# Genomics-HSE/VGsim

Measured on AMD Instinct MI355X. Metric: simulated events/sec (direct + tau-leap) at 1/2/4/8 MI355X vs Cython CPU, higher is better.
Workload: dtype f64; 1 GPU; BASELINE config 3: 65536 haplotypes (8 sites) x 64 populations x 1 susceptibility group, direct Gillespie, bit-exact mode (PCG64 stream, reference summation order), index-case start, b=2.5 d=0.9 s=0.1 m=0.01/site, total migration 0.01, N=1e7; replicates_per_gpu=16384, events_per_replicate=100000, trajectory_points=1001

## Files before the change

vgsim_amd/csrc/vgx_quad.hip:

```cpp
#include <hip/hip_runtime.h>
#include <stdint.h>
#include <vector>
#include "vgx_dev.h"
#include "vgx_rng.h"
#include "vgx_wave.h"
#include "vgx_rowprim.h"
#include "vgx_rowlist.h"
#include "vgx_flat.h"

#ifndef VGX_QUAD_WAVES
#define VGX_QUAD_WAVES 2
#endif

#ifdef VGX_PROFILE
#define QPROF(i)                                                        \
    do {                                                                \
        unsigned long long prof_t1 = __builtin_readcyclecounter();      \
        prof_acc[i] += prof_t1 - prof_t0;                               \
        prof_t0 = prof_t1;                                              \
    } while (0)
#else
#define QPROF(i)
#endif

// ... 226 lines not shown
}

extern "C" __global__ void __launch_bounds__(64) vgx_quad_prep_kernel(VgxDevParams p, const double *cd, double *effMig,
                                                                     double *maxEBM, int32_t *has_mig) {
    const int P = p.P;
    bool anyf = false;
    for (int base = 0; base < P; base += 64) {
        const int pn2 = base + (int)threadIdx.x;
        double mx = 0.0;
        if (pn2 < P) {
            const double *m2 = p.mig + (int64_t)pn2 * P;
            for (int pn1 = 0; pn1 < P; ++pn1) {
                if (pn1 == pn2) continue;
                const double *m1 = p.mig + (int64_t)pn1 * P;
                double e = 0.0;
                for (int pn3 = 0; pn3 < P; ++pn3) e += m1[pn3] * m2[pn3] * cd[pn3] / p.actualSizes[pn3];
                effMig[(int64_t)pn1 * P + pn2] = e;
                if (e > mx) mx = e;
            }
            maxEBM[pn2] = mx * p.maxEffectiveBirth;
        }
        anyf = anyf || (__ballot(pn2 < P && mx * p.maxEffectiveBirth != 0.0) != 0ull);
    }
    if (threadIdx.x == 0) *has_mig = anyf ? 1 : 0;
}
extern "C" __attribute__((visibility("hidden"))) hipError_t vgxi_launch_quad_prep(const VgxDevParams *p, const double *cd, double *effMig,
                                                                                 double *maxEBM, int32_t *has_mig, hipStream_t stream) {
    hipLaunchKernelGGL(vgx_quad_prep_kernel, dim3(1), dim3(64), 0, stream, *p, cd, effMig, maxEBM, has_mig);
    return hipGetLastError();
}

struct VgxQuadKArgs { VgxDirectArgs a; QArgs qa; };
typedef const VgxQuadKArgs __attribute__((address_space(4))) *QuadKA;
template <int QT, bool RCPDIV>
static __device__ __forceinline__ void quad_body() {
    const QuadKA ka = (QuadKA)__builtin_amdgcn_kernarg_segment_ptr();
    const auto &a = ka->a;
    const auto &qa = ka->qa;
    const int lane = threadIdx.x, row = lane >> 4, rl = lane & 15;
    const auto &p = a.p;
    const auto &r = a.r;
    const int P = p.P, sites = p.sites, H = p.H;
    const int64_t R = a.n_replicates;
    const int64_t rep_raw = (int64_t)blockIdx.x * 4 + row;
    const bool live = rep_raw < R;
    const int64_t rep = live ? rep_raw : R - 1;
    const int nslot = (P + 15) >> 4;
    const bool has_mig = qa.has_mig[0] != 0;

    extern __shared__ __attribute__((aligned(16))) unsigned char smem[];
    double *k_cd = (double *)smem, *k_as = k_cd + 64, *k_smul = k_as + 64, *k_mebm = k_smul + 64, *k_rcp = k_mebm + 64;
    uint64_t *k_jump = (uint64_t *)(smem + Q_CONST_BYTES) + rl * 4;
    unsigned char *blk = smem + Q_CONST_BYTES + Q_RNG_BYTES + row * Q_REP_BYTES;
    double *s_inf = (double *)blk, *s_bc = s_inf + 64;
    double *s_ts = s_bc + 64, *s_ti = s_ts + 64;
    int32_t *s_nocc = (int32_t *)(s_ti + 64);
    double *s_cc = (double *)(s_nocc + 64);
    int64_t *s_cnt = (int64_t *)(s_cc + 4);
    uint64_t *s_inc = (uint64_t *)(s_cnt + 6);
    int32_t *s_zero = (int32_t *)(s_inc + 2);
    uint32_t *s_stage = (uint32_t *)(s_zero + 64);
    int stage_n = 0;
    int64_t stage_slot0 = 0;
    auto stage_flush = [&](bool f) {
        WSYNC();
        if (f && live) {
            const int n6 = stage_n * 6;
            int32_t *c = r.ev_cols + (rep * r.evcap + stage_slot0) * VGX_EV_COLS;
            uint32_t *q = (uint32_t *)(r.ev_rate + rep * r.evcap + stage_slot0);
#pragma unroll
            for (int j = 0; j < 3; ++j)
                if (rl + 16 * j < n6) c[rl + 16 * j] = (int32_t)s_stage[rl + 16 * j];
            if (rl < 2 * stage_n) q[rl] = s_stage[48 + rl];
        }
        if (f) stage_n = 0;
        WSYNC();
    };
#define QBUMP(i) do { if (rl == 0) s_cnt[i] += 1; } while (0)

    const double c_b = p.cb_b[0], c_sig = p.cb_sigma[0], c_d = p.c_d[0], c_s = p.c_s[0], c_tm = p.c_tm[0];

    {
        const double *gD = r.popD + rep * PD_COUNT * P;
        const int64_t *gI64 = r.popI + rep * PI_COUNT * P;
        const int32_t *gN = r.nocc + rep * P;
        const int pn = lane;
        k_cd[pn] = pn < P ? gD[PD_CD * P + pn] : 0.0;
        k_as[pn] = pn < P ? p.actualSizes[pn] : 1.0;
        k_rcp[pn] = pn < P ? 1.0 / p.actualSizes[pn] : 1.0;
        k_smul[pn] = pn < P ? c_s * p.sampMult[pn] : 0.0;
        k_mebm[pn] = pn < P ? qa.maxEBM[pn] : 0.0;
        for (int s = 0; s < 4; ++s) {
            const int pq = s * 16 + rl;
            const bool ok = pq < P;
            s_inf[pq] = 0.0; s_bc[pq] = 0.0;
            if (rl < 4) s_cc[rl] = 0.0;
            s_ts[pq] = ok ? (double)gI64[PI_TOTSUS * P + pq] : 0.0;
            s_ti[pq] = ok ? (double)gI64[PI_TOTINF * P + pq] : 0.0;
            s_nocc[pq] = ok ? gN[pq] : 0;
            s_zero[pq] = QT < 4 && ok ? gN[pq] : 0;
        }
    }
    WSYNC();

    const int64_t cap = r.cap, capT = r.capT;
    int32_t *lhap = r.lhap + rep * P * cap;
    int32_t *lcls = r.lcls + rep * P * cap;
    int64_t *lcnt = r.lcnt + rep * P * cap;
    int32_t *lcnt32 = r.lcnt32 + rep * P * cap;
#define L8(pop) ((uint8_t *)(r.lcnt32 + R * P * cap) + (rep * P + (int64_t)(pop)) * cap)
#define B8(v) ((uint8_t)((v) < 255 ? (v) : 255))
    int64_t *ltsum = r.ltsum + rep * P * capT;
    const bool has_traj = r.traj != nullptr;
    const VgxRepScalars *sc = r.sc + rep;
    if (QT < 4) {
        for (int pn = 0; pn < P; ++pn) q_zero_tail(lcnt32 + (int64_t)pn * cap, s_nocc[pn], cap, live);
        WSYNC();
    }

    double t_now = sc->currentTime, totalRate = 0.0, totalMig = 0.0;
    double gI = (double)sc->globalInfectious;
    int64_t ev_ptr = sc->ev_ptr;
    int64_t cS = sc->sCounter;
    if (rl == 0) {
        s_cnt[QC_B] = sc->bCounter; s_cnt[QC_D] = sc->dCounter; s_cnt[QC_M] = sc->mCounter;
        s_cnt[QC_MIGP] = sc->migPlus; s_cnt[QC_MIGN] = sc->migNonPlus;
    }
    int64_t loops = 0, att_loops = 0, good_attempt = sc->good_attempt;
    int att = 0, restarts = 0, last_att = -1, traj_next = 0;
    int st = live ? ST_REBUILD : ST_DONE, err = 0;
    bool open = false;
    const double tlimit = (double)a.time;
    const bool has_tl = !(a.time == -1.0f);

    if (row == 0) {
        const uint64_t MH = 0x2360ED051FC65DA4ull, ML = 0x4385DF649FCCF645ull;
        uint64_t Ah = MH, Al = ML, Gh = 0, Gl = 1;
        for (int j = 1; j < 16; ++j) {
            uint64_t nh, nl, gh, gl;
            vgx_mul128(Ah, Al, MH, ML, nh, nl);
            vgx_mul128(Gh, Gl, MH, ML, gh, gl);
            vgx_add128(gh, gl, 0, 1);
            if (j <= rl) { Ah = nh; Al = nl; Gh = gh; Gl = gl; }
        }
        k_jump[0] = Ah; k_jump[1] = Al; k_jump[2] = Gh; k_jump[3] = Gl;
    }
    WSYNC();
    uint64_t g_sh = 0, g_sl = 0;
    double g_val = 0.0;
    int pos = 8;
    int32_t ch_cn[4] = {0, 0, 0, 0};
    double tc = 0.0;
    int tc_pi = -1;

#ifdef VGX_PROFILE
    unsigned long long prof_acc[VGX_PROF_SLOTS], prof_t0 = __builtin_readcyclecounter();
    for (int i = 0; i < VGX_PROF_SLOTS; ++i) prof_acc[i] = 0;
    int prof_tiles[13] = {0, 0, 0, 0, 0, 0, 0, 0, 0, 0, 0, 0, 0};
#endif
    while (true) {
        QPROF(0);
        const bool run = st != ST_DONE;
        if (!__ballot(run)) break;
        const bool rebuild = st == ST_REBUILD;

        bool end_attempt = false, ev = false;
        if (st == ST_RUN) {
            if (!open) {
                if (att >= a.attempts) {
                    st = ST_DONE;
                } else {
                    VgxPcg64 sd;
                    vgx_pcg64_seed(sd, (uint64_t)r.seeds[rep], (uint32_t)att);
                    g_sh = sd.sh; g_sl = sd.sl;
                    if (rl == 0) { s_inc[0] = sd.ih; s_inc[1] = sd.il; }
                    pos = 8;
                    open = true;
                    last_att = att; att_loops = 0;
                    if (!(totalRate + totalMig != 0.0 && gI != 0.0)) end_attempt = true;
                }
            }
            if (st == ST_RUN && !end_attempt &&
                !(ev_ptr < a.ev_size && (a.sample_size == -1 || cS <= a.sample_size) && (!has_tl || t_now < tlimit)))
                end_attempt = true;
            if (st == ST_RUN && !end_attempt) {
                if (loops >= a.max_loop) { err = Q_ERR_LOOP_GUARD; st = ST_DONE; }
                else ev = true;
            }
        }

        int u_lo = 0, u_hi = rebuild ? P : 0;
        int op_n = 0, op_pi = 0, op_h0 = 0, op_h1 = 0;
        int op_d0 = 0;
        int e_type = -1, e_hap = 0, e_pop = 0, e_nh = 0, e_np = 0;
        double den = 0.0;
        int ch_pi = -1;
        double m_pre[4] = {0.0, 0.0, 0.0, 0.0};
        int pm_pi = -1;

        QPROF(1);
        if (__ballot(ev)) {
            if (__builtin_expect(__ballot(ev && pos == 8) != 0, 0)) {
                const bool fill = ev && pos == 8;
                uint64_t h, l, ch, cl;
                vgx_mul128(k_jump[0], k_jump[1], g_sh, g_sl, h, l);
                vgx_mul128(k_jump[2], k_jump[3], s_inc[0], s_inc[1], ch, cl);
                vgx_add128(h, l, ch, cl);
                const double u = vgx_pcg64_output_double(h, l);
                const double v = (rl & 1) ? u : -vgx_log(u);
                const uint64_t nh = (uint64_t)rowget_i64((int64_t)h, 15), nl = (uint64_t)rowget_i64((int64_t)l, 15);
                if (fill) { g_val = v; g_sh = nh; g_sl = nl; pos = 0; }
            }
            const int pp = min(pos, 7);
            const double nlog = rowget_f64(g_val, 2 * pp), u2 = rowget_f64(g_val, 2 * pp + 1);
            if (ev) { pos += 1; loops += 1; att_loops += 1; }
            QPROF(2);
            den = totalRate + totalMig;
            const double t_new = t_now + (nlog / den);
            if (has_traj) {
                while (true) {
                    const double tg = r.traj_t0 + (double)traj_next * r.traj_dt;
                    const bool emit = ev && live && traj_next < r.traj_points && tg < t_new;
                    if (__builtin_expect(!__ballot(emit), 1)) break;
                    if (emit) {
                        double *o = r.traj + (rep * r.traj_points + traj_next) * (int64_t)P * 2;
                        for (int s = 0; s < nslot; ++s) {
                            const int pn = s * 16 + rl;
                            if (pn < P) { o[pn * 2 + 0] = s_ti[pn]; o[pn * 2 + 1] = s_ts[pn]; }
                        }
                        traj_next += 1;
                    }
                }
            }
            if (ev) t_now = t_new;

            QPROF(3);
            double rn = u2;
            const double choose0 = rn * den;
            double choose = choose0;
            const bool evn = ev && (totalRate > choose);
            const bool evm = ev && !evn;

            int pi = 0;
            {
                rn = choose / totalRate;
                const double rr_ = totalRate * rn;
                const double c0 = s_cc[0], c1 = s_cc[1], c2 = s_cc[2], c3 = s_cc[3];
                const int slot = !(c0 < rr_) ? 0 : !(c1 < rr_) ? 1 : !(c2 < rr_) ? 2 : 3;
                const bool any = !(c3 < rr_);
                const double cin = slot == 0 ? 0.0 : slot == 1 ? c0 : slot == 2 ? c1 : c2;
                const double w = s_inf[slot * 16 + rl];
                double tot_;
                const double pre = row_scan16(w, cin, tot_);
                const int q = row_min(any && slot * 16 + rl < P && !(pre < rr_) ? rl : 16);
                double total, wi;
                if (q < 16) { pi = slot * 16 + q; total = rowget_f64(pre, q); wi = rowget_f64(w, q); }
                else { pi = P - 1; total = c3; wi = s_inf[P - 1]; }
                if (evn && wi == 0.0) err = Q_ERR_ZERO_WEIGHT + 256 * 1;
                rn = (rr_ - (total - wi)) / wi;
                choose = rn * wi;
            }
            const double infect_pi = s_inf[pi];
            rn = (choose - 0.0) / infect_pi;
            const double bC = s_bc[pi];
            const double smul = k_smul[pi];
            const double tE = ((bC + c_d) + smul) + c_tm;
            const int n_sel = evn ? s_nocc[pi] : 0;
            const int32_t *lh = lhap + (int64_t)pi * cap;
            int32_t *l3 = lcnt32 + (int64_t)pi * cap;
            int64_t *lt = ltsum + (int64_t)pi * capT;
            {
                const double *mrow = p.mig + (int64_t)pi * P;
#pragma unroll
                for (int s = 0; s < 4; ++s)
                    if (s < nslot) m_pre[s] = mrow[min(s * 16 + rl, P - 1)];
                pm_pi = evn ? pi : -1;
            }

            QPROF(4);
            const double r2 = infect_pi * rn;
            int k_hit = -1;
            double pre_hit = 0.0, w_hit = 0.0;
            int hap_hit = 0;
            int64_t cnt_hit = 0;
            const int maxn = rows_max(n_sel);
            if (__builtin_expect(maxn <= 64, QT < 4)) {
                const int nch = (maxn + 15) >> 4;
                const int last = max(n_sel - 1, 0);
                const double tEz = n_sel > 0 ? tE : 0.0;
                int32_t cn4[4];
                int hp4[4];
                double w4[4];
#pragma unroll
                for (int c = 0; c < 4; ++c) {
                    cn4[c] = 0; hp4[c] = 0; w4[c] = 0.0;
                    if (c < nch) {
                        const int k = c * 16 + rl;
                        hp4[c] = lh[min(k, last)];
                        if (QT < 4 && c > 0) {
                            cn4[c] = l3[k];
                            w4[c] = tEz * (double)cn4[c];
                        } else {
                            cn4[c] = l3[min(k, last)];
                            w4[c] = k < n_sel ? tE * (double)cn4[c] : 0.0;
                        }
                    }
                }
                double carry = 0.0, carry_hit = 0.0;
                int c_hit = nch == 1 ? 0 : -1;
                if (nch > 1) {
#pragma unroll
                    for (int c = 0; c < 4; ++c) {
                        if (c < nch) {
                            const double acc = row_sum16(w4[c], carry);
                            if (c_hit < 0 && c * 16 < n_sel && !(acc < r2)) { c_hit = c; carry_hit = carry; }
                            carry = acc;
                        }
                    }
                }
                const int cc = c_hit >= 0 ? c_hit : (last >> 4);
                const double w = cc == 0 ? w4[0] : cc == 1 ? w4[1] : cc == 2 ? w4[2] : w4[3];
                const int32_t cn = cc == 0 ? cn4[0] : cc == 1 ? cn4[1] : cc == 2 ? cn4[2] : cn4[3];
                const int hp = cc == 0 ? hp4[0] : cc == 1 ? hp4[1] : cc == 2 ? hp4[2] : hp4[3];
                double tot_;
                const double pre = row_scan16(w, c_hit >= 0 ? carry_hit : 0.0, tot_);
                if (nch == 1) carry = tot_;
                const int q = row_min(c_hit >= 0 && cc * 16 + rl < n_sel && !(pre < r2) ? rl : 16);
                const int qq = q < 16 ? q : (last & 15);
                pre_hit = q < 16 ? rowget_f64(pre, qq) : carry;
                w_hit = rowget_f64(w, qq);
                hap_hit = rowget_i32(hp, qq); cnt_hit = rowget_i32(cn, qq);
                if (q < 16) k_hit = cc * 16 + q;
                else if (evn) {
                    if (n_sel > 0 && hap_hit == H - 1 && (QT < 4 || cnt_hit != 0)) k_hit = n_sel - 1; else err = Q_ERR_ZERO_WEIGHT + 256 * 2;
                }
                if (evn) {
#pragma unroll
                    for (int c = 0; c < 4; ++c) ch_cn[c] = cn4[c];
                    ch_pi = pi;
                }
            } else {
#ifdef VGX_PROFILE
                prof_acc[15] += 1;
#endif
#ifdef VGX_PROFILE
                if (QT < 4) {
                    const bool hit_ = n_sel > 64 && tc_pi == pi, miss_ = n_sel > 64 && tc_pi != pi;
                    prof_tiles[7] += hit_; prof_tiles[8] += miss_;
                    if (!__ballot(miss_) && row == 0) prof_tiles[9] += 1;
                    prof_tiles[10] += n_sel > 256; prof_tiles[11] += n_sel > 512;
                    if (__ballot(n_sel > 0 && n_sel <= 64) && row == 0) prof_tiles[12] += 1;
                }
#endif
                QSel sel;
                q_long_select<QT>(l3, lh, n_sel, maxn, tE, r2, evn, H, sel, (double *)(ltsum + (int64_t)pi * capT + R * P * capT) ,
                                  pi, tc, tc_pi);
                k_hit = sel.k_hit; pre_hit = sel.pre_hit; w_hit = sel.w_hit; hap_hit = sel.hap_hit; cnt_hit = sel.cnt_hit;
                if (sel.err) err = sel.err;
#ifdef VGX_PROFILE
                {
                    const int nt_ = (n_sel + 63) >> 6, need_ = k_hit >= 0 ? (k_hit >> 6) + 1 : nt_;
                    prof_tiles[0] += nt_; prof_tiles[1] += (maxn + 63) >> 6; prof_tiles[2] += need_; prof_tiles[3] += rows_max(need_);
                }
#endif
            }
            const bool evn_ok = evn && err == 0;
            if (evn && w_hit == 0.0 && err == 0) err = Q_ERR_ZERO_WEIGHT + 256 * 4;
            rn = (r2 - (pre_hit - w_hit)) / w_hit;

            QPROF(5);
            int ei = 0;
            {
                const double r3 = tE * rn;
                double total = bC, wi = bC;
                if (total < r3) { ei = 1; total += c_d; wi = c_d; }
                if (ei == 1 && total < r3) { ei = 2; total += smul; wi = smul; }
                if (ei == 2 && total < r3) { ei = 3; total += c_tm; wi = c_tm; }
                if (evn_ok && wi == 0.0) err = Q_ERR_ZERO_WEIGHT + 256 * 5;
                rn = (r3 - (total - wi)) / wi;
            }
            const bool go = evn && err == 0;
            const double ts_pi = s_ts[pi], ti_pi = s_ti[pi];
            const bool isB = go && ei == 0, isD = go && (ei == 1 || ei == 2), isM = go && ei == 3;
            if (isB) {
                if (ts_pi * c_sig == 0.0) err = Q_ERR_ZERO_WEIGHT + 256 * 6;
                if (rl == 0) { s_ts[pi] = ts_pi - 1.0; s_ti[pi] = ti_pi + 1.0; }
                gI += 1.0; QBUMP(QC_B);
                if (live && rl == 0) { l3[k_hit] = (int32_t)(cnt_hit + 1); if (QT >= 4) { L8(pi)[k_hit] = B8(cnt_hit + 1); if (n_sel > 64) lt[k_hit >> 6] += 1; } }
                if (QT >= 4 || maxn <= 64) {
#pragma unroll
                    for (int c = 0; c < 4; ++c)
                        if (c == (k_hit >> 4) && rl == (k_hit & 15)) ch_cn[c] += 1;
                }
                e_type = QEV_BIRTH; e_hap = hap_hit; e_pop = pi; e_nh = 0; e_np = H;
                u_lo = pi; u_hi = pi + 1;
            }
            if (isD) {
                if (rl == 0) { s_ts[pi] = ts_pi + 1.0; s_ti[pi] = ti_pi - 1.0; }
                gI -= 1.0;
                if (ei == 2) { cS += 1; e_type = QEV_SAMPLING; } else { QBUMP(QC_D); e_type = QEV_DEATH; }
                if (QT < 4 && cnt_hit == 1) { op_n = 1; op_pi = pi; op_h0 = hap_hit; op_d0 = -1; ch_pi = -1; }
                else {
                    if (live && rl == 0) { l3[k_hit] = (int32_t)(cnt_hit - 1); if (QT >= 4) { L8(pi)[k_hit] = B8(cnt_hit - 1); if (n_sel > 64) lt[k_hit >> 6] -= 1; } }
                    if (QT >= 4 && cnt_hit == 1 && rl == 0) s_zero[pi] += 1;
                    if (QT >= 4 || maxn <= 64) {
#pragma unroll
                        for (int c = 0; c < 4; ++c)
                            if (c == (k_hit >> 4) && rl == (k_hit & 15)) ch_cn[c] -= 1;
                    }
                }
                e_hap = hap_hit; e_pop = pi; e_nh = 0; e_np = 0;
                u_lo = pi; u_hi = pi + 1;
            }
            QPROF(6);
            if (__builtin_expect(__ballot(isM) != 0, 0)) {
                const double *mr = p.mRate + (int64_t)hap_hit * sites;
                int mi = 0;
                {
                    const double rq = c_tm * rn;
                    double total = isM ? mr[0] : 1.0, wi = total;
                    for (int i = 1; i < sites; ++i) {
                        if (isM && mi == i - 1 && total < rq) { mi = i; wi = mr[i]; total += wi; }
                    }
                    if (isM && wi == 0.0) err = Q_ERR_ZERO_WEIGHT + 256 * 7;
                    rn = (rq - (total - wi)) / wi;
                }
                const double *hm = p.hapMutType + ((int64_t)hap_hit * sites + mi) * 3;
                int DS = 0;
                if (isM) {
                    const double h0 = hm[0], h1 = hm[1], h2 = hm[2];
                    const double rq = ((h0 + h1) + h2) * rn;
                    double total = h0, wi = h0;
                    if (total < rq) { DS = 1; total += h1; wi = h1; }
                    if (DS == 1 && total < rq) { DS = 2; total += h2; wi = h2; }
                    if (wi == 0.0) err = Q_ERR_ZERO_WEIGHT + 256 * 8;
                }
                if (isM && err == 0) {
                    const int digit4 = 1 << (2 * (sites - mi - 1));
                    const int AS = (hap_hit / digit4) % 4;
                    if (DS >= AS) DS += 1;
                    const int nhi = hap_hit + (DS - AS) * digit4;
                    if (QT >= 4) {
                        if (live && rl == 0) { l3[k_hit] = (int32_t)(cnt_hit - 1); L8(pi)[k_hit] = B8(cnt_hit - 1); if (n_sel > 64) lt[k_hit >> 6] -= 1; if (cnt_hit == 1) s_zero[pi] += 1; }
                        op_n = 1; op_pi = pi; op_h0 = nhi; op_d0 = +1; ch_pi = -1;
                    } else {
                        op_n = 2; op_pi = pi; op_h0 = nhi; op_d0 = +1; op_h1 = hap_hit; ch_pi = -1;
                    }
                    QBUMP(QC_M);
                    e_type = QEV_MUTATION; e_hap = hap_hit; e_pop = pi; e_nh = nhi; e_np = 0;
                    u_lo = pi; u_hi = pi + 1;
                }
            }
            QPROF(7);
            if (__builtin_expect(__ballot(evm) != 0, 0)) {
                double rm = (choose0 - totalRate) / totalMig;
                int tpi = 0;
                {
                    const double rr_ = totalMig * rm;
                    double carry = 0.0, tot_hit = 0.0, w_h = 0.0;
                    int cand = 64;
                    for (int s = 0; s < nslot; ++s) {
                        const int pn = s * 16 + rl;
                        const double w = pn < P ? k_mebm[pn] * s_ts[pn] * (gI - s_ti[pn]) : 0.0;
                        double tot_;
                        const double pre = row_scan16(w, carry, tot_);
                        const int q = row_min(cand == 64 && pn < P && !(pre < rr_) ? rl : 16);
                        if (cand == 64 && q < 16) { cand = s * 16 + q; tot_hit = rowget_f64(pre, q); w_h = rowget_f64(w, q); }
                        else if (s == nslot - 1 && cand == 64) {
                            const int ql = (P - 1) & 15;
                            tot_hit = rowget_f64(pre, ql); w_h = rowget_f64(w, ql);
                        }
                        carry = tot_;
                    }
                    tpi = cand < 64 ? cand : P - 1;
                    if (evm && w_h == 0.0) err = Q_ERR_ZERO_WEIGHT + 256 * 9;
                    rm = (rr_ - (tot_hit - w_h)) / w_h;
                }
                int spi = -1;
                {
                    const double rr_ = (gI - s_ti[tpi]) * rm;
                    const int start = tpi == 0 ? 1 : 0;
                    int64_t carry = 0, total = 0;
                    for (int s = 0; s < nslot; ++s) {
                        const int pn = s * 16 + rl;
                        const bool in = pn < P && pn != tpi && pn >= start;
                        const int64_t w = in ? (int64_t)s_ti[pn] : 0;
                        const int64_t pre = row_iscan(w) + carry;
                        const int q = row_min(spi < 0 && in && !((double)pre < rr_) ? rl : 16);
                        if (spi < 0 && q < 16) { spi = s * 16 + q; total = rowget_i64(pre, q); }
                        carry = rowget_i64(pre, 15);
                    }
                    if (spi < 0) { spi = P - 1; total = carry; }
                    const int64_t wi = (int64_t)s_ti[spi];
                    if (evm && wi == 0) err = Q_ERR_ZERO_WEIGHT + 256 * 10;
                    rm = (rr_ - (double)(total - wi)) / (double)wi;
                }
                int hi = 0;
                {
                    const int n = evm ? s_nocc[spi] : 0;
                    const int32_t *lh2 = lhap + (int64_t)spi * cap;
                    const int32_t *l32 = lcnt32 + (int64_t)spi * cap;
#define CN2(k) ((int64_t)l32[k])
                    const int64_t *lt2 = ltsum + (int64_t)spi * capT;
                    const double rr_ = s_ti[spi] * rm;
                    int64_t before = 0;
                    int base = 0;
                    bool none = false;
                    const int maxn2 = rows_max(n);
                    if (__builtin_expect(maxn2 > 64, QT >= 4)) {
                        const int nt = n > 64 ? (n + 63) >> 6 : 0;
                        const int maxt = rows_max(nt);
                        int jt = -1;
                        int64_t carry = 0;
                        if (QT < 4) {
                            for (int t = 0; t < maxt; ++t) {
                                const QTile c = tile_load(l32, t < nt ? t : 0, rl);
                                const int64_t w = t < nt ? (int64_t)c.c0 + (int64_t)c.c1 + (int64_t)c.c2 + (int64_t)c.c3 : 0;
                                const int64_t pre = rowget_i64(row_iscan(w), 15) + carry;
                                if (jt < 0 && t < nt && !((double)pre < rr_)) { jt = t; before = carry; }
                                carry = pre;
                                if (!__ballot(jt < 0 && t + 1 < nt)) break;
                            }
                        } else
                        for (int tb = 0; tb < maxt; tb += 16) {
                            const int j = tb + rl;
                            const int64_t w = j < nt ? lt2[j] : 0;
                            const int64_t pre = row_iscan(w) + carry;
                            const int q = row_min(jt < 0 && j < nt && !((double)pre < rr_) ? rl : 16);
                            if (jt < 0 && q < 16) { jt = tb + q; before = rowget_i64(pre, q) - rowget_i64(w, q); }
                            carry = rowget_i64(pre, 15);
                        }
                        if (nt > 0) { if (jt < 0) { none = true; before = carry; } else base = jt * 64; }
                    }
                    int kq = -1;
                    int64_t total = before, wi = 0;
// ... 104 lines not shown
                    if (stride >= 16 && maxn <= stride) continue;
                    const int k = lo + rl * stride;
                    const int h = (act && k < n) ? lh[k] : 0x7fffffff;
                    const int nle = row_min(h <= hap ? 16 : rl);
                    if (stride == 1) {
                        const int q = row_min(h >= hap ? rl : 16);
                        posn = lo + q;
                        if (posn > n) posn = n;
                        const int hq = rowget_i32(h, min(q, 15));
                        found = q < 16 && hq == hap;
                    } else {
                        lo = lo + (nle > 0 ? (nle - 1) * stride : 0);
                    }
                }
                if (act && found) cur = l3[posn];
            }
            const bool bump = act && found && cur + delta != 0;
            const bool rem = act && found && cur + delta == 0;
            const bool ins = act && !found;
            if (ins && n >= cap) { err = Q_ERR_CAPACITY; }
            const bool ins_ok = ins && err == 0;
            if (bump && rl == 0) l3[posn] = cur + delta;
            if (__builtin_expect(__ballot(ins_ok) != 0, 0)) {
                enum { SU = 4 };
                int hi_ = ins_ok ? n : 0;
                const int lo_ = ins_ok ? posn : 0;
                while (__ballot(hi_ > lo_)) {
                    const int blo = max(lo_, hi_ - SU * 16);
                    int h[SU];
                    int32_t ct[SU];
#pragma unroll
                    for (int u = 0; u < SU; ++u) {
                        const int k = blo + u * 16 + rl;
                        h[u] = 0; ct[u] = 0;
                        if (k < hi_) { h[u] = lh[k]; ct[u] = l3[k]; }
                    }
                    WSYNC();
#pragma unroll
                    for (int u = 0; u < SU; ++u) {
                        const int k = blo + u * 16 + rl;
                        if (k < hi_) { lh[k + 1] = h[u]; lc[k + 1] = 0; l3[k + 1] = ct[u]; }
                    }
                    WSYNC();
                    hi_ = blo;
                }
                if (ins_ok && rl == 0) { lh[posn] = hap; lc[posn] = 0; l3[posn] = delta; s_nocc[op_pi] = n + 1; if (n + 1 > s_zero[op_pi]) s_zero[op_pi] = n + 1; }
                q_zero_tail(l3, n + 1, cap, ins_ok && ((n + 1) & 63) == 0);
                WSYNC();
            }
            if (__builtin_expect(__ballot(rem) != 0, 0)) {
                enum { SU = 4 };
                int lo_ = rem ? posn + 1 : 0;
                const int hi_ = rem ? n : 0;
                while (__ballot(lo_ < hi_)) {
                    int h[SU];
                    int32_t ct[SU];
#pragma unroll
                    for (int u = 0; u < SU; ++u) {
                        const int k = lo_ + u * 16 + rl;
                        h[u] = 0; ct[u] = 0;
                        if (k < hi_) { h[u] = lh[k]; ct[u] = l3[k]; }
                    }
                    WSYNC();
#pragma unroll
                    for (int u = 0; u < SU; ++u) {
                        const int k = lo_ + u * 16 + rl;
                        if (k < hi_) { lh[k - 1] = h[u]; l3[k - 1] = ct[u]; }
                    }
                    WSYNC();
                    lo_ += SU * 16;
                }
                if (rem && rl == 0) { s_nocc[op_pi] = n - 1; l3[n - 1] = 0; }
                WSYNC();
            }
        }

        QPROF(9);
        if (err == 0 && e_type >= 0) {
            if (a.record_events) {
                const int64_t slot = ev_ptr - r.ev_base;
                if (slot >= 0 && slot < r.evcap) {
                    if (stage_n == 0) stage_slot0 = slot;
                    if (rl < 8) {
                        const int v = rl == 0 ? e_type : rl == 1 ? e_hap : rl == 2 ? e_pop : rl == 3 ? e_nh : rl == 4 ? e_np
                                      : rl == 5 ? (int)(uint32_t)att_loops : rl == 6 ? __double2loint(den) : __double2hiint(den);
                        s_stage[rl < 6 ? stage_n * 6 + rl : 48 + 2 * stage_n + (rl - 6)] = (uint32_t)v;
                    }
                    stage_n += 1;
                } else {
                    err = Q_ERR_CAPACITY;
                }
            }
            ev_ptr += 1;
        }
        if (__builtin_expect(__ballot(stage_n == 8) != 0, 0)) stage_flush(stage_n == 8);

        QPROF(10);
        if (err != 0) u_hi = u_lo;
        const int maxu = rows_max(u_hi - u_lo);
        if (maxu > 0) {
            for (int us = 0; us < maxu; ++us) {
                const int pn0 = u_lo + us;
                const bool act = pn0 < u_hi;
                const int pi = act ? pn0 : 0;
                const double x = s_ts[pi] * c_sig;
                const double *mrow = p.mig + (int64_t)pi * P;
                const bool mhave = act && pi == pm_pi;
                double tv4[4], ps = 0.0;
#pragma unroll
                for (int s = 0; s < 4; ++s) {
                    tv4[s] = 0.0;
                    if (s < nslot) {
                        const int pn = s * 16 + rl;
                        const double m = mhave ? m_pre[s] : mrow[min(pn, P - 1)];
                        const double t = x * m * m * k_cd[pn];
                        tv4[s] = RCPDIV ? div_by_const(t, k_as[pn], k_rcp[pn]) : t / k_as[pn];
                        if (QT >= 4 && pn >= P) tv4[s] = 0.0;
                    }
                }
#pragma unroll
                for (int s = 0; s < 4; ++s)
                    if (s < nslot) ps = row_sum16(tv4[s], ps);
                const double bC = c_b * ps;
                const double tE = ((bC + c_d) + k_smul[pi]) + c_tm;
                QPROF(11);
                const int n = act ? s_nocc[pi] : 0;
                const int32_t *l3 = lcnt32 + (int64_t)pi * cap;
                const int maxn = rows_max(n);
                double acc = 0.0;
                if (__builtin_expect(maxn <= 64, QT < 4)) {
                    const int nch = (maxn + 15) >> 4;
                    const bool chave = act && pi == ch_pi;
                    if (QT < 4 && act && pi == tc_pi) tc_pi = -1;
                    const double tEz = n > 0 ? tE : 0.0;
                    int32_t cn4[4];
#pragma unroll
                    for (int c = 0; c < 4; ++c) cn4[c] = ch_cn[c];
                    if (__ballot(act && !chave)) {
                        const int last = max(n - 1, 0);
#pragma unroll
                        for (int c = 0; c < 4; ++c)
                            if (c < nch) { const int32_t cl = l3[QT < 4 && c > 0 ? c * 16 + rl : min(c * 16 + rl, last)]; if (!chave) cn4[c] = cl; }
                    }
#pragma unroll
                    for (int c = 0; c < 4; ++c)
                        if (c < nch) acc = row_sum16(QT < 4 && c > 0 ? tEz * (double)cn4[c] : c * 16 + rl < n ? tE * (double)cn4[c] : 0.0, acc);
                } else {
#ifdef VGX_PROFILE
                    prof_tiles[4] += (n + 63) >> 6; prof_tiles[5] += (maxn + 63) >> 6; prof_tiles[6] += 1;
#endif
                    acc = q_long_sum<QT>(l3, L8(pi), n, maxn, tE, (double *)(ltsum + (int64_t)pi * capT + R * P * capT), act, pi, tc, tc_pi);
                }
                if (act && rl == 0) { s_bc[pi] = bC; s_inf[pi] = acc; }
                WSYNC();
                QPROF(12);
            }
            {
                double w4[4], carry = 0.0, cend[4];
#pragma unroll
                for (int s = 0; s < 4; ++s) w4[s] = s_inf[s * 16 + rl];
#pragma unroll
                for (int s = 0; s < 4; ++s) {
                    if (s < nslot) carry = row_sum16(w4[s], carry);
                    cend[s] = carry;
                }
                if (u_hi > u_lo) {
                    if (rl < 4) s_cc[rl] = rl == 0 ? cend[0] : rl == 1 ? cend[1] : rl == 2 ? cend[2] : cend[3];
                    totalRate = carry;
                }
                WSYNC();
            }
            QPROF(13);
            if (has_mig) {
                double w4[4], acc = 0.0;
#pragma unroll
                for (int s = 0; s < 4; ++s) {
                    w4[s] = 0.0;
                    if (s < nslot) {
                        const int pn = s * 16 + rl;
                        w4[s] = k_mebm[pn] * s_ts[pn] * (gI - s_ti[pn]);
                        if (QT >= 4 && pn >= P) w4[s] = 0.0;
                    }
                }
#pragma unroll
                for (int s = 0; s < 4; ++s)
                    if (s < nslot) acc = row_sum16(w4[s], acc);
                if (u_hi > u_lo) totalMig = acc;
            }
        }

        QPROF(14);
        if (rebuild && st == ST_REBUILD) st = err ? ST_DONE : ST_RUN;
        if (err != 0) st = ST_DONE;
        if (ev && st == ST_RUN && (totalRate == 0.0 || gI == 0.0)) end_attempt = true;
        if (st == ST_RUN && end_attempt) {
            open = false;
            if (ev_ptr <= 100 && a.iterations > 100) {
                ev_ptr = 0; cS = 0;
                stage_n = 0;
                if (rl < 6) s_cnt[rl] = 0;
                t_now = 0.0; traj_next = 0;
                restarts += 1; att += 1;
                st = ST_REBUILD;
                tc_pi = -1;
            } else {
                good_attempt = (int64_t)att + 1;
                st = ST_DONE;
            }
        }
        if (__builtin_expect(__ballot(st == ST_REBUILD && restarts > 0 && !rebuild) != 0, 0)) {
            const bool rs = st == ST_REBUILD && restarts > 0 && !rebuild && live;
            int64_t g = 0;
            for (int pn = 0; pn < P; ++pn) {
                const int n = r.i_nocc[pn];
                const int n_old = rs ? s_nocc[pn] : 0;
                int64_t ti = 0;
                for (int base = 0; base < n; base += 64) {
                    int64_t tsum = 0;
                    for (int c4 = 0; c4 < 4; ++c4) {
                        const int k = base + c4 * 16 + rl;
                        int64_t ct = 0;
                        if (k < n) {
                            ct = r.i_cnt[(int64_t)pn * r.i_cap + k];
                            if (rs) {
                                lhap[(int64_t)pn * cap + k] = r.i_hap[(int64_t)pn * r.i_cap + k];
                                lcls[(int64_t)pn * cap + k] = r.i_cls[(int64_t)pn * r.i_cap + k];
                                if (QT >= 4) lcnt[(int64_t)pn * cap + k] = ct;
                                lcnt32[(int64_t)pn * cap + k] = (int32_t)ct;
                                if (QT >= 4) L8(pn)[k] = B8(ct);
                            }
                        }
                        tsum += rowget_i64(row_iscan(ct), 15);
                    }
                    if (rs && rl == 0) ltsum[(int64_t)pn * capT + base / 64] = tsum;
                    ti += tsum;
                }
                if (rs)
                    for (int j = (n + 63) / 64 + rl; j <= n_old / 64 && j < capT; j += 16) ltsum[(int64_t)pn * capT + j] = 0;
                if (QT < 4) q_zero_tail(lcnt32 + (int64_t)pn * cap, n, cap, rs);
                if (rs && rl == 0) { s_nocc[pn] = n; if (QT >= 4) s_zero[pn] = 0; else if (n > s_zero[pn]) s_zero[pn] = n; s_ts[pn] = (double)r.i_sus[pn]; s_ti[pn] = (double)ti; }
                g += ti;
            }
            if (rs) gI = (double)g;
            WSYNC();
        }
    }

    if (has_traj) {
        while (true) {
            const bool emit = live && traj_next < r.traj_points;
            if (!__ballot(emit)) break;
            if (emit) {
                double *o = r.traj + (rep * r.traj_points + traj_next) * (int64_t)P * 2;
                for (int s = 0; s < nslot; ++s) {
                    const int pn = s * 16 + rl;
                    if (pn < P) { o[pn * 2 + 0] = s_ti[pn]; o[pn * 2 + 1] = s_ts[pn]; }
                }
                traj_next += 1;
            }
        }
    }

#ifdef VGX_PROFILE
    if (lane == 0 && r.prof)
        for (int i = 0; i < VGX_PROF_SLOTS; ++i) r.prof[rep * VGX_PROF_SLOTS + i] = prof_acc[i];
    for (int i = 0; i < 13; ++i) {
        const long long t4 = (long long)__builtin_amdgcn_readlane(prof_tiles[i], 0) + __builtin_amdgcn_readlane(prof_tiles[i], 16) +
                             __builtin_amdgcn_readlane(prof_tiles[i], 32) + __builtin_amdgcn_readlane(prof_tiles[i], 48);
        if (lane == 0 && r.prof && rep_raw + 1 < R) r.prof[(rep_raw + 1) * VGX_PROF_SLOTS + i] = (unsigned long long)t4;
    }
#endif
    stage_flush(stage_n > 0);
    WSYNC();
    if (QT < 4) {
        for (int pn = 0; pn < P; ++pn) {
            const int n = live ? s_nocc[pn] : 0, top = live ? s_zero[pn] : 0;
            const int32_t *l3 = lcnt32 + (int64_t)pn * cap;
            const int jmax = rows_max(top >> 6);
            for (int j = 0; j <= jmax && j < capT; ++j) {
                int64_t w = 0;
#pragma unroll
                for (int i = 0; i < 4; ++i) {
                    const int k = j * 64 + 4 * rl + i;
                    if (k < n) w += (int64_t)l3[k];
                }
                const int64_t tsum = rowget_i64(row_iscan(w), 15);
                if (live && rl == 0 && j <= (top >> 6)) ltsum[(int64_t)pn * capT + j] = tsum;
            }
        }
    }
    if (live) {
        double *gD = r.popD + rep * PD_COUNT * P;
        int64_t *gI64 = r.popI + rep * PI_COUNT * P;
        int32_t *gN = r.nocc + rep * P;
        VgxRepScalars *sc = r.sc + rep;
        for (int s = 0; s < nslot; ++s) {
            const int pn = s * 16 + rl;
            if (pn < P) {
                gD[PD_POPRATE * P + pn] = s_inf[pn];
                gD[PD_INFECT * P + pn] = s_inf[pn];
                gD[PD_IMMUNE * P + pn] = 0.0;
                gD[PD_MIG * P + pn] = k_mebm[pn] * s_ts[pn] * (gI - s_ti[pn]);
                gD[PD_MAXEBM * P + pn] = k_mebm[pn];
                gI64[PI_TOTSUS * P + pn] = (int64_t)s_ts[pn];
                gI64[PI_TOTINF * P + pn] = (int64_t)s_ti[pn];
                gN[pn] = s_nocc[pn];
                r.sus[rep * P + pn] = (int64_t)s_ts[pn];
                r.immSrc[rep * P + pn] = 0.0;
            }
        }
        if (rl == 0) {
            sc->currentTime = t_now; sc->totalRate = totalRate; sc->totalMig = totalMig;
            sc->globalInfectious = (int64_t)gI;
            sc->bCounter = s_cnt[QC_B]; sc->dCounter = s_cnt[QC_D]; sc->sCounter = cS; sc->mCounter = s_cnt[QC_M];
            sc->migPlus = s_cnt[QC_MIGP]; sc->migNonPlus = s_cnt[QC_MIGN];
            sc->good_attempt = good_attempt;
            sc->ev_ptr = ev_ptr; sc->loop_iterations = loops; sc->restarts = restarts;
            sc->loc_n = 0; sc->error = err; sc->traj_next = traj_next;
            sc->last_attempt = last_att; sc->last_attempt_loops = att_loops;
            sc->fa_n = 0;
        }
    }
}

#ifndef VGX_QT_SHORT
#define VGX_QT_SHORT 1
#endif
extern "C" __global__ void __launch_bounds__(64, VGX_QUAD_WAVES) vgx_quad_kernel(VgxQuadKArgs) { quad_body<VGX_QT_SHORT, true>(); }
#ifndef VGX_QT_LONG
#define VGX_QT_LONG 7
#endif
extern "C" __global__ void __launch_bounds__(64, VGX_QUAD_WAVES) vgx_quad_long_kernel(VgxQuadKArgs) { quad_body<VGX_QT_LONG, true>(); }
extern "C" __global__ void __launch_bounds__(64, VGX_QUAD_WAVES) vgx_quad_kernel_plaindiv(VgxQuadKArgs) { quad_body<VGX_QT_SHORT, false>(); }
extern "C" __global__ void __launch_bounds__(64, VGX_QUAD_WAVES) vgx_quad_long_kernel_plaindiv(VgxQuadKArgs) { quad_body<VGX_QT_LONG, false>(); }

extern "C" __global__ void __launch_bounds__(256) vgx_quad_counts32_kernel(const int64_t *c64, int32_t *c32, int64_t n) {
    for (int64_t i = (int64_t)blockIdx.x * 256 + threadIdx.x; i < n; i += (int64_t)gridDim.x * 256) c32[i] = (int32_t)c64[i];
}
extern "C" __attribute__((visibility("hidden"))) hipError_t vgxi_launch_counts32(const int64_t *c64, int32_t *c32, int64_t n, hipStream_t stream) {
    hipLaunchKernelGGL(vgx_quad_counts32_kernel, dim3(4096), dim3(256), 0, stream, c64, c32, n);
    return hipGetLastError();
}

extern "C" __global__ void __launch_bounds__(256) vgx_quad_counts8_kernel(const int32_t *c32, uint8_t *c8, int64_t n4) {
    for (int64_t i = (int64_t)blockIdx.x * 256 + threadIdx.x; i < n4; i += (int64_t)gridDim.x * 256) {
        const int4 v = *(const int4 *)(c32 + 4 * i);
        *(uint32_t *)(c8 + 4 * i) = (uint32_t)min(max(v.x, 0), 255) | ((uint32_t)min(max(v.y, 0), 255) << 8) | ((uint32_t)min(max(v.z, 0), 255) << 16) |
                                    ((uint32_t)min(max(v.w, 0), 255) << 24);
    }
}

extern "C" __global__ void __launch_bounds__(256) vgx_traj_i32_kernel(const double *src, int32_t *dst, int64_t n) {
    for (int64_t i = (int64_t)blockIdx.x * 256 + threadIdx.x; i < n; i += (int64_t)gridDim.x * 256) dst[i] = (int32_t)src[i];
}
extern "C" __attribute__((visibility("hidden"))) hipError_t vgxi_launch_traj_i32(const double *src, int32_t *dst, int64_t n, hipStream_t stream) {
    hipLaunchKernelGGL(vgx_traj_i32_kernel, dim3(8192), dim3(256), 0, stream, src, dst, n);
    return hipGetLastError();
// ... 125 lines not shown
```

Before: 1.145 billion events/s.

## Keep per-population infection weights and prefix sums in registers for small-QT path

For the QT<4 template path, per-lane copies of the infection weights (inf4) and the slot prefix sums (cc4) are kept in registers, so the population selection no longer reads s_inf and s_cc from shared memory. One wave sync after the weight update is dropped on that path. The per-event termination checks are also replaced by a countdown of guaranteed-safe events, so the full condition is re-evaluated only when the budget runs out. This adds register pressure and depends on the register copies staying consistent with shared memory across rebuilds and restarts.

```diff
diff --git a/vgsim_amd/csrc/vgx_quad.hip b/vgsim_amd/csrc/vgx_quad.hip
--- a/vgsim_amd/csrc/vgx_quad.hip
+++ b/vgsim_amd/csrc/vgx_quad.hip
@@ -402,6 +402,8 @@
     int32_t ch_cn[4] = {0, 0, 0, 0};
     double tc = 0.0;
     int tc_pi = -1;
+    double inf4[4] = {0.0, 0.0, 0.0, 0.0}, cc4[4] = {0.0, 0.0, 0.0, 0.0};
+    int safe = 0;
 
 #ifdef VGX_PROFILE
     unsigned long long prof_acc[VGX_PROF_SLOTS], prof_t0 = __builtin_readcyclecounter();
@@ -430,12 +432,36 @@
                     if (!(totalRate + totalMig != 0.0 && gI != 0.0)) end_attempt = true;
                 }
             }
-            if (st == ST_RUN && !end_attempt &&
-                !(ev_ptr < a.ev_size && (a.sample_size == -1 || cS <= a.sample_size) && (!has_tl || t_now < tlimit)))
-                end_attempt = true;
-            if (st == ST_RUN && !end_attempt) {
-                if (loops >= a.max_loop) { err = Q_ERR_LOOP_GUARD; st = ST_DONE; }
-                else ev = true;
+            if (QT >= 4) {
+                if (st == ST_RUN && !end_attempt &&
+                    !(ev_ptr < a.ev_size && (a.sample_size == -1 || cS <= a.sample_size) && (!has_tl || t_now < tlimit)))
+                    end_attempt = true;
+                if (st == ST_RUN && !end_attempt) {
+                    if (loops >= a.max_loop) { err = Q_ERR_LOOP_GUARD; st = ST_DONE; }
+                    else ev = true;
+                }
+            }
+        }
+        if (QT < 4) {
+            const bool chk = st == ST_RUN && !end_attempt;
+            bool slow = false;
+            if (__builtin_expect(__ballot(chk && safe <= 0) != 0, 0)) {
+                if (chk && safe <= 0) {
+                    int64_t m = min(a.ev_size - ev_ptr, a.max_loop - loops);
+                    if (a.sample_size != -1) m = min(m, a.sample_size - cS + 1);
+                    safe = (int)max(min(m, (int64_t)0x7fffffff), (int64_t)0);
+                    if (safe == 0) {
+                        slow = true;
+                        if (!(ev_ptr < a.ev_size && (a.sample_size == -1 || cS <= a.sample_size) && (!has_tl || t_now < tlimit)))
+                            end_attempt = true;
+                        else if (loops >= a.max_loop) { err = Q_ERR_LOOP_GUARD; st = ST_DONE; }
+                        else ev = true;
+                    }
+                }
+            }
+            if (chk && !slow) {
+                safe -= 1;
+                if (has_tl && !(t_now < tlimit)) end_attempt = true; else ev = true;
             }
         }
 
@@ -492,28 +518,48 @@
             const bool evm = ev && !evn;
 
             int pi = 0;
+            double infect_pi = 0.0;
             {
                 rn = choose / totalRate;
                 const double rr_ = totalRate * rn;
-                const double c0 = s_cc[0], c1 = s_cc[1], c2 = s_cc[2], c3 = s_cc[3];
-                const int slot = !(c0 < rr_) ? 0 : !(c1 < rr_) ? 1 : !(c2 < rr_) ? 2 : 3;
-                const bool any = !(c3 < rr_);
-                const double cin = slot == 0 ? 0.0 : slot == 1 ? c0 : slot == 2 ? c1 : c2;
-                const double w = s_inf[slot * 16 + rl];
-                double tot_;
-                const double pre = row_scan16(w, cin, tot_);
-                const int q = row_min(any && slot * 16 + rl < P && !(pre < rr_) ? rl : 16);
                 double total, wi;
-                if (q < 16) { pi = slot * 16 + q; total = rowget_f64(pre, q); wi = rowget_f64(w, q); }
-                else { pi = P - 1; total = c3; wi = s_inf[P - 1]; }
+                if (QT < 4) {
+                    const double c0 = cc4[0], c1 = cc4[1], c2 = cc4[2], c3 = cc4[3];
+                    const bool any = !(c3 < rr_);
+                    const int slot = !any ? nslot - 1 : !(c0 < rr_) ? 0 : !(c1 < rr_) ? 1 : !(c2 < rr_) ? 2 : 3;
+                    const double cin = slot == 0 ? 0.0 : slot == 1 ? c0 : slot == 2 ? c1 : c2;
+                    const double w = slot == 0 ? inf4[0] : slot == 1 ? inf4[1] : slot == 2 ? inf4[2] : inf4[3];
+                    double tot_;
+                    const double pre = row_scan16(w, cin, tot_);
+                    const int q = row_min(any && slot * 16 + rl < P && !(pre < rr_) ? rl : 16);
+                    const int qq = q < 16 ? q : (P - 1) & 15;
+                    pi = q < 16 ? slot * 16 + q : P - 1;
+                    const double tq = rowget_f64(pre, qq);
+                    wi = rowget_f64(w, qq);
+                    total = q < 16 ? tq : c3;
+                } else {
+                    const double c0 = s_cc[0], c1 = s_cc[1], c2 = s_cc[2], c3 = s_cc[3];
+                    const int slot = !(c0 < rr_) ? 0 : !(c1 < rr_) ? 1 : !(c2 < rr_) ? 2 : 3;
+                    const bool any = !(c3 < rr_);
+                    const double cin = slot == 0 ? 0.0 : slot == 1 ? c0 : slot == 2 ? c1 : c2;
+                    const double w = s_inf[slot * 16 + rl];
+                    double tot_;
+                    const double pre = row_scan16(w, cin, tot_);
+                    const int q = row_min(any && slot * 16 + rl < P && !(pre < rr_) ? rl : 16);
+                    if (q < 16) { pi = slot * 16 + q; total = rowget_f64(pre, q); wi = rowget_f64(w, q); }
+                    else { pi = P - 1; total = c3; wi = s_inf[P - 1]; }
+                }
                 if (evn && wi == 0.0) err = Q_ERR_ZERO_WEIGHT + 256 * 1;
                 rn = (rr_ - (total - wi)) / wi;
                 choose = rn * wi;
-            }
-            const double infect_pi = s_inf[pi];
+                infect_pi = wi;
+            }
+            if (QT >= 4) infect_pi = s_inf[pi];
             rn = (choose - 0.0) / infect_pi;
             const double bC = s_bc[pi];
             const double smul = k_smul[pi];
+            double ts_pi = 0.0, ti_pi = 0.0;
+            if (QT < 4) { ts_pi = s_ts[pi]; ti_pi = s_ti[pi]; }
             const double tE = ((bC + c_d) + smul) + c_tm;
             const int n_sel = evn ? s_nocc[pi] : 0;
             const int32_t *lh = lhap + (int64_t)pi * cap;
@@ -630,7 +676,7 @@
                 rn = (r3 - (total - wi)) / wi;
             }
             const bool go = evn && err == 0;
-            const double ts_pi = s_ts[pi], ti_pi = s_ti[pi];
+            if (QT >= 4) { ts_pi = s_ts[pi]; ti_pi = s_ti[pi]; }
             const bool isB = go && ei == 0, isD = go && (ei == 1 || ei == 2), isM = go && ei == 3;
             if (isB) {
                 if (ts_pi * c_sig == 0.0) err = Q_ERR_ZERO_WEIGHT + 256 * 6;
@@ -1041,20 +1087,27 @@
                     acc = q_long_sum<QT>(l3, L8(pi), n, maxn, tE, (double *)(ltsum + (int64_t)pi * capT + R * P * capT), act, pi, tc, tc_pi);
                 }
                 if (act && rl == 0) { s_bc[pi] = bC; s_inf[pi] = acc; }
-                WSYNC();
+                if (QT < 4) {
+#pragma unroll
+                    for (int s = 0; s < 4; ++s)
+                        if (act && pi == s * 16 + rl) inf4[s] = acc;
+                } else WSYNC();
                 QPROF(12);
             }
             {
                 double w4[4], carry = 0.0, cend[4];
 #pragma unroll
-                for (int s = 0; s < 4; ++s) w4[s] = s_inf[s * 16 + rl];
+                for (int s = 0; s < 4; ++s) w4[s] = QT < 4 ? inf4[s] : s_inf[s * 16 + rl];
 #pragma unroll
                 for (int s = 0; s < 4; ++s) {
                     if (s < nslot) carry = row_sum16(w4[s], carry);
                     cend[s] = carry;
                 }
                 if (u_hi > u_lo) {
-                    if (rl < 4) s_cc[rl] = rl == 0 ? cend[0] : rl == 1 ? cend[1] : rl == 2 ? cend[2] : cend[3];
+                    if (QT < 4) {
+#pragma unroll
+                        for (int s = 0; s < 4; ++s) cc4[s] = cend[s];
+                    } else if (rl < 4) s_cc[rl] = rl == 0 ? cend[0] : rl == 1 ? cend[1] : rl == 2 ? cend[2] : cend[3];
                     totalRate = carry;
                 }
                 WSYNC();
@@ -1092,6 +1145,7 @@
                 restarts += 1; att += 1;
                 st = ST_REBUILD;
                 tc_pi = -1;
+                safe = 0;
             } else {
                 good_attempt = (int64_t)att + 1;
                 st = ST_DONE;
```

New measurement: 1.163 billion events/s (median of 6 runs). +1.6%, better.
